# MatteoGiuseppetti/Hybrid-Autoencoder-MLP-Pipeline-for-Satellite-Image-Classification

Measured on AMD Instinct MI355X. Metric: EuroSAT 64x64 RGB images/sec (AE+MLP train step), higher is better.
Workload: dtype bf16; 1 GPU; BASELINE configs[2]: joint conv-AE + classification head train step (fwd, 35*MSE+CE, bwd, Adam), 64x64x3 inputs, 64-d latent, bf16 storage / fp32 accumulate; per_gpu_batch=512, global_batch=512, parallelism=single

## Files before the change

### hybrid-autoencoder-mlp-pipeline-for-satellite-image-classification_amd/csrc/eae_ctx.h

```cpp
#pragma once
#include "eae_internal.h"
#include "eae_args.h"
#include <atomic>
#include <functional>
#include <vector>

#define RC(x) do { int rc__ = (x); if (rc__) return rc__; } while (0)

constexpr float BN_EPS = 1e-5f, BN_MOM = 0.1f;
const int ENC_C[5] = {3, 32, 64, 128, 256};
const int BN_C[7] = {32, 64, 128, 256, 128, 64, 32};
const int BN_GAMMA_IDX[7] = {2, 6, 10, 14, 22, 26, 30};
const int W3_PARAM[6] = {4, 8, 12, 20, 24, 28};
const int W3_A[6] = {64, 128, 256, 256, 128, 64};
const int W3_B[6] = {32, 64, 128, 128, 64, 32};
const int PREBN_BIAS[7] = {1, 5, 9, 13, 21, 25, 29};

struct eae_ctx {
  eae_config cfg;
  int H, W, L, C, Bm;
  int Cin = 3, CP = 4;
  int Lp = 0;
  bool lpad = false;
  float *gs_encw = nullptr, *gs_encb = nullptr, *gs_decw = nullptr, *gs_head = nullptr, *zstage = nullptr;
  size_t pk_w1p = 0, pk_bep = 0;
  bool fp8 = false;
  size_t pk8_p1[6] = {}, pk8_p2[6] = {};
  Fp8State* q = nullptr;
  float* bn_save = nullptr;
  long long Pn, K;
  long long poff[39], bnoff[15];
  float *P = nullptr, *G = nullptr, *M = nullptr, *V = nullptr, *bnrun = nullptr;
  long long* nbt = nullptr;
  long long adam_step = 0;
  bool packed = false;
  bool fwd_ready = false;
  bool fwd_eval_ready = false;
  bool has_enc = true, has_dec = true;
  int enc_ready = 0, dec_ready = 0;
  bool bwd_eval = false;
  bool prebn_dirty = false;
  int fwd_B = 0, fwd_head = 0;
  const float* fwd_x = nullptr;
  long long fwd_gen = 0;
  void* ws = nullptr;
  bf16_t *y[4], *u[3], *d0, *gy[4], *gu[3], *gd0, *g4;
  bf16_t *dyy[4], *dyu[3];
  float *z, *dz, *dzc, *coef_f[7], *coef_b[7], *stat, *wscratch, *fcpart, *msepart, *cepart, *headpart, *lossbuf;
  long long wscratch_floats, head_stride;
  uint8_t* pack = nullptr;
// ... 80 lines not shown
  bool clip_on() const { return clip_max != 0.f; }
  float* dyn = nullptr;
  static constexpr int PROF_RING = 64;
  bool prof_on = false;
  int prof_site = 0;
  int prof_n = 0;
  hipEvent_t prof_ev[3 * PROF_RING] = {};
  EaeProfHook prof_hook = {};
  long long act_elems(int lvl) const {
    return (long long)(H >> lvl) * (W >> lvl) * ENC_C[lvl];
  }
};

inline void invalidate_forward(eae_ctx* c) { c->fwd_ready = false; c->fwd_eval_ready = false; c->enc_ready = 0; c->dec_ready = 0; }
inline long long r4(long long n) { return (n + 3) & ~3LL; }
inline unsigned* poison_word(const eae_ctx* c) { return reinterpret_cast<unsigned*>(c->acc_base + c->poison_off); }
inline SrcDesc src_raw(const bf16_t* p) { SrcDesc s; s.p0 = p; s.p1 = nullptr; s.coef = nullptr; return s; }
inline SrcDesc src_bnrelu(const bf16_t* y, const float* coef) { SrcDesc s; s.p0 = y; s.p1 = nullptr; s.coef = coef; return s; }
inline SrcDesc src_bnbwd(const bf16_t* g, const bf16_t* y, const float* coef) { SrcDesc s; s.p0 = g; s.p1 = y; s.coef = coef; return s; }
inline SrcDesc src_f32(const float* p) { SrcDesc s; s.p0 = reinterpret_cast<const bf16_t*>(p); s.p1 = nullptr; s.coef = nullptr; return s; }

extern const unsigned EV_FLAGS;

void sq_push(eae_ctx* c, std::function<int(hipStream_t, float*)> f, int pin = -1);
void sq_fork(eae_ctx* c);
void take_sig(eae_ctx* c, ConvArgs& a);
int sq_commit(eae_ctx* c, hipStream_t st);
int fold_side2(eae_ctx* c);
int join_side_begin(eae_ctx* c, hipStream_t st, GateArgs* g);
int join_side(eae_ctx* c, hipStream_t st);
int streams_distinct(eae_ctx* c, hipStream_t user);
// ... 17 lines not shown
```

### hybrid-autoencoder-mlp-pipeline-for-satellite-image-classification_amd/csrc/eae_ctx.hip

```cpp
#include "eae_ctx.h"
#include <string>
#include <cstring>
#include <cstdlib>

static thread_local std::string g_err;
int eae_set_error(int code, const char* msg) { g_err = msg ? msg : "unknown error"; return code; }
extern "C" const char* eae_last_error(void) { return g_err.c_str(); }
extern "C" int eae_version(void) { return 100; }

const unsigned EV_FLAGS = hipEventDisableTiming | (getenv("EAE_EVENT_SYSTEM_FENCE") ? 0u : hipEventDisableSystemFence);

namespace {

int bands_of(const eae_config& c) { return c.in_channels == 0 ? 3 : c.in_channels; }

void param_sizes(const eae_config& c, long long* sz) {
  const long long P = (long long)(c.image_h / 16) * (c.image_w / 16), K = 256 * P, L = c.latent_dim, C = c.num_classes;
  const long long N = bands_of(c);
  const long long s[38] = {32 * 9 * N, 32, 32, 32, 64 * 32 * 9, 64, 64, 64, 128 * 64 * 9, 128, 128, 128, 256 * 128 * 9, 256, 256, 256,
                           L * K, L, K * L, K, 256 * 128 * 9, 128, 128, 128, 128 * 64 * 9, 64, 64, 64, 64 * 32 * 9, 32, 32, 32,
                           32 * 9 * N, N, 128 * L, 128, C * 128, C};
  for (int i = 0; i < 38; ++i) sz[i] = s[i];
}

// ... 126 lines not shown
  const long long LK = c->Lp * c->K;
  c->pk_we1 = pcarve(LK * 2); add(c->poff[16], c->pk_we1, LK, PACK_FC_ROWMAJOR_KPERM, c->Lp, 256, (int)c->Pn, 0);
  c->pk_we2 = pcarve(LK * 2); add(c->poff[16], c->pk_we2, LK, PACK_FC_TRANS_KPERM, c->Lp, 256, (int)c->Pn, 0);
  c->pk_wd1 = pcarve(LK * 2); add(c->poff[18], c->pk_wd1, LK, PACK_FC_ROWPERM, c->Lp, 256, (int)c->Pn, 0);
  c->pk_wd2 = pcarve(LK * 2); add(c->poff[18], c->pk_wd2, LK, PACK_FC_ROWPERM_TRANS, c->Lp, 256, (int)c->Pn, 0);
  for (int k = 0; k < 4; ++k) descs[descs.size() - 1 - k].lv = c->L;
  if (c->lpad) {
    c->pk_w1p = pcarve(128LL * c->Lp * 4); add(c->poff[34], c->pk_w1p, 128LL * c->Lp, PACK_PAD_COLS, c->Lp, 0, 0, 1); descs.back().lv = c->L;
    c->pk_bep = pcarve(c->Lp * 4); add(c->poff[17], c->pk_bep, c->Lp, PACK_PAD_COLS, c->Lp, 0, 0, 1); descs.back().lv = c->L;
  }
  c->pk_bd = pcarve(c->K * 4); add(c->poff[19], c->pk_bd, c->K, PACK_FC_ROWPERM, 1, 256, (int)c->Pn, 1);
  c->ndesc = (int)descs.size();
  std::vector<unsigned short> blkmap(descs.size() * 1024);
  c->blk_tot = eae_pack_assign_blocks(descs.data(), (int)descs.size(), blkmap.data(), (int)blkmap.size());
  c->pack_bytes = poffb;
  size_t o_pack = carve(poffb), o_desc = carve(descs.size() * sizeof(PackDesc)), o_q = carve(sizeof(Fp8State)), o_bns = carve(2048 * 4 + 64);
  size_t o_bmap = carve((size_t)(c->blk_tot > 0 ? c->blk_tot : 1) * sizeof(unsigned short));
  hipError_t e = hipMalloc(&c->ws, off);
  if (e != hipSuccess) { delete c; return eae_set_error(EAE_ERR_HIP, hipGetErrorString(e)); }
  uint8_t* b = static_cast<uint8_t*>(c->ws);
  for (int i = 0; i < 4; ++i) { c->y[i] = (bf16_t*)(b + o_y[i]); c->gy[i] = (bf16_t*)(b + o_gy[i]); }
  for (int i = 0; i < 3; ++i) {
    c->u[i] = (bf16_t*)(b + o_u[i]); c->gu[i] = (bf16_t*)(b + o_gu[i]);
    c->dyu[i] = ((dy_mask_env >> (4 + i)) & 1u) ? (bf16_t*)(b + o_dyu[i]) : nullptr;
  }
  c->dyy[0] = nullptr;
  for (int i = 1; i < 4; ++i) c->dyy[i] = ((dy_mask_env >> i) & 1u) ? (bf16_t*)(b + o_dyy[i]) : nullptr;
  c->d0 = (bf16_t*)(b + o_d0); c->gd0 = (bf16_t*)(b + o_gd0); c->g4 = (bf16_t*)(b + o_g4);
  c->z = (float*)(b + o_z); c->dz = (float*)(b + o_dz); c->dzc = (float*)(b + o_dzc);
  if (c->lpad) {
// ... 13 lines not shown
  c->sigwords = (unsigned*)(b + o_sig);
  c->q = (Fp8State*)(b + o_q);
  c->bn_save = (float*)(b + o_bns);
  {
    Fp8State h;
    eae_fp8_state_init(&h);
    hipError_t eq = hipMemcpy(c->q, &h, sizeof(h), hipMemcpyHostToDevice);
    if (eq != hipSuccess) { hipFree(c->ws); delete c; return eae_set_error(EAE_ERR_HIP, hipGetErrorString(eq)); }
  }
  const char* rcc = getenv("ROCPROF_COUNTER_COLLECTION");
  c->use_gates = getenv("EAE_FORK_EVENTS") == nullptr && !(rcc && atoi(rcc) != 0);
  if (const char* gt = getenv("EAE_GATE_TIMEOUT_MS")) c->gate_limit = (unsigned long long)(atof(gt) * 1e5);
  c->use_graph = getenv("EAE_GRAPH") != nullptr;
  e = hipMemcpy(c->descs_dev, descs.data(), descs.size() * sizeof(PackDesc), hipMemcpyHostToDevice);
  if (e == hipSuccess && c->blk_tot > 0) e = hipMemcpy(c->blkmap, blkmap.data(), (size_t)c->blk_tot * sizeof(unsigned short), hipMemcpyHostToDevice);
  if (e == hipSuccess) e = hipMemset(c->g4, 0, Bm * (size_t)c->H * c->W * c->CP * 2);
  if (e == hipSuccess && c->lpad) e = hipMemset(c->zstage, 0, Bm * (size_t)c->Lp * 4);
  if (e == hipSuccess) e = hipMemset(c->z, 0, Bm * (size_t)c->Lp * 4);
  if (e == hipSuccess) e = hipMemset(c->dz, 0, Bm * (size_t)c->Lp * 4);
  if (e == hipSuccess) e = hipMemset(c->acc_base, 0, c->acc_bytes);
  if (e == hipSuccess) e = hipMemset(c->sigwords, 0, 64);
  c->acc_clean = true; c->bwd_dirty = false;
  c->dy_mask = (getenv("EAE_DY_MASK") ? (unsigned)strtoul(getenv("EAE_DY_MASK"), nullptr, 0) : 0u) & 0x3cu;
  c->skip_wgrad = getenv("EAE_SKIP_WGRAD") != nullptr;
  c->nan_exact = (getenv("EAE_NAN_EXACT") && atoi(getenv("EAE_NAN_EXACT")) != 0) ? 1 : 0;
  c->fold_fwd = getenv("EAE_NO_FOLD_FWD") == nullptr;
  c->fold_bwd = getenv("EAE_NO_FOLD_BWD") == nullptr;
  if (e != hipSuccess) { hipFree(c->ws); delete c; return eae_set_error(EAE_ERR_HIP, hipGetErrorString(e)); }
  c->use_side = getenv("EAE_NO_SIDE_STREAM") == nullptr && cfg->side_streams >= 0;
  if (c->use_side) {
// ... 224 lines not shown
```

### hybrid-autoencoder-mlp-pipeline-for-satellite-image-classification_amd/csrc/eae_dp.hip

```cpp
#include "eae_ctx.h"
#include "eae_common.hip.h"
#include <chrono>
#include <cstring>
#include <cstdlib>
#include <future>
#include <memory>
#include <string>
#include <thread>
#include <dlfcn.h>
#include <rccl/rccl.h>
namespace {
struct RcclApi {
  void* h = nullptr;
  decltype(&ncclGetUniqueId) getUniqueId = nullptr;
  decltype(&ncclCommInitRank) commInitRank = nullptr;
  decltype(&ncclCommDestroy) commDestroy = nullptr;
  decltype(&ncclAllReduce) allReduce = nullptr;
  decltype(&ncclBroadcast) broadcast = nullptr;
  decltype(&ncclGetErrorString) getErrorString = nullptr;
  decltype(&ncclGroupStart) groupStart = nullptr;
  decltype(&ncclGroupEnd) groupEnd = nullptr;
  std::string err;
};
RcclApi* rccl_api() {
// ... 132 lines not shown
    EAE_HIP(hipEventRecord(c->ev_dp_done, c->dp_stream[0]));
  }
  if (grp) RCCL(r->groupStart(), "ncclGroupStart");
  {
    int rc = eae_dp_allreduce_bucket(c, st, 0, ov ? cut : total);
    if (!rc) {
      ncclResult_t e = r->allReduce(flag, flag, 2, ncclUint32, ncclMax, static_cast<ncclComm_t>(c->dp_comm), st);
      if (e != ncclSuccess) rc = rccl_fail(r, e, "ncclAllReduce (flag)");
    }
    if (grp) { ncclResult_t e = r->groupEnd(); if (!rc && e != ncclSuccess) rc = rccl_fail(r, e, "ncclGroupEnd"); }
    RC(rc);
  }
  if (ov) EAE_HIP(hipStreamWaitEvent(st, c->ev_dp_done, 0));
  RC(launch_adam(c, st, c->poff[38], lr, 0.f, 1.0f / (float)c->dp_world, flag, flag + 1));
  c->last_loss = nullptr;
  c->packed = false; c->acc_clean = true; c->bwd_dirty = false;
  return 0;
}
```

### hybrid-autoencoder-mlp-pipeline-for-satellite-image-classification_amd/csrc/eae_misc.h

```cpp
#pragma once
#include <hip/hip_runtime.h>
#include <stdint.h>

enum { PACK_COPY = 0, PACK_3x3_P1, PACK_3x3_P2, PACK_K27, PACK_DECONV4_JOINT, PACK_FC_ROWMAJOR_KPERM, PACK_FC_TRANS_KPERM,
       PACK_FC_ROWPERM, PACK_FC_ROWPERM_TRANS, PACK_KCP, PACK_PAD_COLS };

struct PackDesc {
  long long src_off;
  long long dst_off;
  long long count;
  int mode, d0, d1, d2;
  int out_f32;
  int lv;
  int q_layer;
  int blk0, nblk;
};

constexpr int FP8_AMAX_SLOTS = 64;
constexpr int FP8_AMAX_STRIDE = 32;
struct Fp8State {
  unsigned amax_act[6][FP8_AMAX_SLOTS * FP8_AMAX_STRIDE];
  unsigned amax_grad[6][FP8_AMAX_SLOTS * FP8_AMAX_STRIDE];
  unsigned amax_w[6][FP8_AMAX_SLOTS * FP8_AMAX_STRIDE];
  float s_act[6], s_grad[6], s_w[6];
// ... 36 lines not shown
                         void* pack_base, Fp8State* q = nullptr, unsigned* clear_word = nullptr);
int eae_launch_adam(hipStream_t st, float* p, const float* g, float* m, float* v, long long n, double lr, double b1, double b2,
                    double eps, double wd, long long step);
constexpr int EAE_CLIP_MAX_PARTS = 512;
struct EaeClip { const double* part; int nparts; float max_norm; float* norm_out; };
int eae_grad_sumsq_parts(long long n);
int eae_launch_grad_sumsq(hipStream_t st, const float* g, const long long* poff39, const long long* sizes38, double* part);
int eae_launch_adam_dyn(hipStream_t st, float* p, const float* g, float* m, float* v, long long n, double b1, double b2, double eps,
                        const float* dyn, const unsigned* bad = nullptr, const unsigned* bad2 = nullptr, float* nan_out = nullptr,
                        const EaeClip* clip = nullptr);
int eae_launch_set_dyn(hipStream_t st, float* dyn, double lr, double b1, double b2, double wd, long long step);
int eae_launch_adam_scaled(hipStream_t st, float* p, const float* g, float* m, float* v, long long n, double lr, double b1, double b2,
                           double eps, double wd, long long step, float gscale, void* zero_buf = nullptr, long long zero_bytes = 0,
                           const unsigned* bad = nullptr, const unsigned* bad2 = nullptr, float* nan_out = nullptr, int nan_fill = 0,
                           int max_blocks = 0 , const EaeClip* clip = nullptr);
int eae_launch_stage_bands(hipStream_t st, const void* src, int elem_bytes, long long N, int C, int H, int W, const long long* index, int B,
                           const float* divisor, float* out, int train, float std, unsigned long long seed, unsigned long long step,
                           const int* params, const float* noise);
int eae_launch_augment(hipStream_t st, const void* in_u8, float* out, int B, int H, int W, int train, float std, unsigned long long seed,
                       unsigned long long step, const int* params, const float* noise);

__device__ __forceinline__ void philox4(uint32_t c0, uint32_t c1, uint32_t c2, uint32_t c3, uint32_t k0, uint32_t k1, uint32_t* o) {
#pragma unroll
  for (int r = 0; r < 10; ++r) {
    uint32_t h0 = __umulhi(0xD2511F53u, c0), l0 = 0xD2511F53u * c0;
    uint32_t h1 = __umulhi(0xCD9E8D57u, c2), l1 = 0xCD9E8D57u * c2;
    uint32_t n0 = h1 ^ c1 ^ k0, n1 = l1, n2 = h0 ^ c3 ^ k1, n3 = l0;
    c0 = n0; c1 = n1; c2 = n2; c3 = n3;
    k0 += 0x9E3779B9u; k1 += 0xBB67AE85u;
  }
// ... 18 lines not shown
```

### hybrid-autoencoder-mlp-pipeline-for-satellite-image-classification_amd/csrc/eae_misc.hip

```cpp
#include "eae_internal.h"
#include "eae_common.hip.h"
#include "eae_misc.h"


__device__ __forceinline__ double wave_sum_f64(double v) {
#pragma unroll
  for (int o = 32; o >= 1; o >>= 1) v += __shfl_xor(v, o, 64);
  return v;
}
__device__ __forceinline__ void reduce_partials_ch(const float* __restrict__ part, int ntiles, int C, int ch, double* red,
                                                   double& a, double& b) {
  const int tid = threadIdx.x;
  const float* p1 = part + (size_t)ch * ntiles;
  const float* p2 = part + ((size_t)C + ch) * ntiles;
  double s1 = 0.0, s2 = 0.0;
  for (int t = tid; t < ntiles; t += 256) { s1 += (double)p1[t]; s2 += (double)p2[t]; }
  s1 = wave_sum_f64(s1); s2 = wave_sum_f64(s2);
  if ((tid & 63) == 0) { red[tid >> 6] = s1; red[4 + (tid >> 6)] = s2; }
  __syncthreads();
  a = ((red[0] + red[1]) + red[2]) + red[3];
  b = ((red[4] + red[5]) + red[6]) + red[7];
}

__global__ EAE_NO_PK __launch_bounds__(256) void bn_finalize_kernel(const float* __restrict__ part, int ntiles, int C, float count,
// ... 136 lines not shown
  const SignalArgs a = group_args<SignalArgs>(gz);
  if (threadIdx.x == 0 && blockIdx.x == 0) __hip_atomic_store(a.word, a.val, __ATOMIC_RELAXED, __HIP_MEMORY_SCOPE_AGENT);
}
int eae_launch_gate(hipStream_t st, const GateArgs& g) {
  eae_launch(gate_kernel, gate_kernel_g, dim3(1), dim3(64), 0, st, g);
  EAE_LAUNCH_CHECK();
  return 0;
}
int eae_launch_signal(hipStream_t st, unsigned* word, unsigned val) {
  const SignalArgs sa = {word, val};
  eae_launch(signal_kernel, signal_kernel_g, dim3(1), dim3(64), 0, st, sa);
  EAE_LAUNCH_CHECK();
  return 0;
}

__device__ __forceinline__ float pack_fetch(const PackDesc& d, const float* __restrict__ src, unsigned i) {
  const unsigned d0 = (unsigned)d.d0, d1 = (unsigned)d.d1, d2 = (unsigned)d.d2;
  switch (d.mode) {
    case PACK_3x3_P1: {
      unsigned b = i % d1, r = i / d1, tap = r % 9u, a = r / 9u;
      return src[(a * d1 + b) * 9u + tap];
    }
    case PACK_3x3_P2: {
      unsigned a = i % d0, r = i / d0, tap = r % 9u, b = r / 9u;
      return src[(a * d1 + b) * 9u + tap];
    }
    case PACK_K27: {
      unsigned k = i & 31u, a = i >> 5;
      if (k >= 27u) return 0.f;
      unsigned tap = k / 3u, c = k % 3u;
      return src[(a * 3u + c) * 9u + tap];
    }
    case PACK_KCP: {
      const unsigned KP = (9u * d2 + 31u) & ~31u, k = i % KP, a = i / KP, tap = k / d2, c = k % d2;
      if (tap >= 9u || c >= d1) return 0.f;
      return src[(a * d1 + c) * 9u + tap];
    }
    case PACK_DECONV4_JOINT: {
      int k = i & 127; int n = i >> 7;
      const int C = (int)d1;
      if (n >= 4 * C) return 0.f;
      int ph = n / C, co = n % C, nb = k >> 5, ci = k & 31;
      int py = ph >> 1, px = ph & 1, dy = nb >> 1, dx = nb & 1;
      int ky = py == 0 ? (dy == 0 ? 1 : -1) : (dy == 0 ? 2 : 0);
      int kx = px == 0 ? (dx == 0 ? 1 : -1) : (dx == 0 ? 2 : 0);
      if (ky < 0 || kx < 0) return 0.f;
      return src[(ci * C + co) * 9 + ky * 3 + kx];
    }
    case PACK_FC_ROWMAJOR_KPERM: {
      unsigned K = d1 * d2, k2 = i % K, r = i / K;
      if (r >= (unsigned)d.lv) return 0.f;
      unsigned c = k2 % d1, p = k2 / d1;
      return src[r * K + c * d2 + p];
    }
    case PACK_FC_TRANS_KPERM: {
      unsigned r = i % d0, k2 = i / d0, K = d1 * d2;
      if (r >= (unsigned)d.lv) return 0.f;
      unsigned c = k2 % d1, p = k2 / d1;
      return src[r * K + c * d2 + p];
    }
    case PACK_FC_ROWPERM: {
      unsigned l = i % d0, j2 = i / d0;
// ... 333 lines not shown
      adam_update(P[j], __builtin_fmaf(G[j], CLIP ? geff : gscale, wp), M[j], V[j], b1, b2, step_size, bc2_sqrt, eps);
    }
    reinterpret_cast<float4*>(p)[i] = pp;
    reinterpret_cast<float4*>(m)[i] = mm;
    reinterpret_cast<float4*>(v)[i] = vv;
  }
}
__global__ EAE_NO_PK __launch_bounds__(256) void adam_kernel(AdamArgs a) { adam_body<false>(a); }
__global__ EAE_NO_PK __launch_bounds__(256) void adam_kernel_g(GroupPack<AdamArgs> p, int gz) { adam_body<false>(group_args<AdamArgs>(gz)); }
__global__ EAE_NO_PK __launch_bounds__(256) void adam_clip_kernel(AdamClipArgs a) { adam_body<true>(a.a, &a.c); }
__global__ EAE_NO_PK __launch_bounds__(256) void adam_clip_kernel_g(GroupPack<AdamClipArgs> p, int gz) {
  const AdamClipArgs a = group_args<AdamClipArgs>(gz);
  adam_body<true>(a.a, &a.c);
}

struct GradNormArgs { const float* g; double* part; unsigned n4; int ntail; unsigned tail[38]; };
__device__ __forceinline__ EAE_NO_PK void grad_sumsq_body(const GradNormArgs& a) {
#pragma clang fp contract(off)
  __shared__ double lds4[4];
  const unsigned T = gridDim.x * 256u, t = blockIdx.x * 256u + threadIdx.x, n4 = a.n4;
  const float4* __restrict__ g4 = reinterpret_cast<const float4*>(a.g);
  double acc = 0.0;
  for (unsigned i0 = t; i0 < n4; i0 += 4u * T) {
    float4 q[4];
#pragma unroll
    for (int u = 0; u < 4; ++u) {
      const unsigned i = i0 + (unsigned)u * T;
      q[u] = g4[i < n4 ? i : n4 - 1];
    }
#pragma unroll
// ... 249 lines not shown
```

### hybrid-autoencoder-mlp-pipeline-for-satellite-image-classification_amd/csrc/eae_step.hip

```cpp
#include "eae_ctx.h"
#include <cmath>
#include <cstdlib>

namespace {

static void prof_hook_begin(void* u, hipStream_t st) {
  eae_ctx* c = static_cast<eae_ctx*>(u);
  hipEventRecord(c->prof_ev[3 * c->prof_n], st);
}
static void prof_hook_end(void* u, hipStream_t st) {
  eae_ctx* c = static_cast<eae_ctx*>(u);
  hipEventRecord(c->prof_ev[3 * c->prof_n + 1], st);
  hipEventRecord(c->prof_ev[3 * c->prof_n + 2], st);
  c->prof_n++;
}
static const EaeProfHook* prof_hook_for(eae_ctx* c, int site) {
  if (!(c->prof_on && c->prof_site == site && c->prof_n < eae_ctx::PROF_RING && !c->capturing)) return nullptr;
  c->prof_hook = EaeProfHook{prof_hook_begin, prof_hook_end, c};
  return &c->prof_hook;
}
struct ProfBracket {
  eae_ctx* c; hipStream_t st; bool on;
  ProfBracket(eae_ctx* c_, int site, hipStream_t st_) : c(c_), st(st_) {
    on = c->prof_on && c->prof_site == site && c->prof_n < eae_ctx::PROF_RING && !c->capturing;
// ... 131 lines not shown
int run_head(eae_ctx* c, hipStream_t st, int B, const long long* labels, float* logits, bool want_grad, const float* dlogits_in,
             bool count_valid = false) {
  HeadArgs h = HeadArgs();
  h.dlogits_in = dlogits_in;
  h.z = c->z; h.w1 = c->lpad ? (const float*)(c->pack + c->pk_w1p) : c->P + c->poff[34]; h.b1 = c->P + c->poff[35]; h.w2 = c->P + c->poff[36]; h.b2 = c->P + c->poff[37];
  h.labels = labels; h.B = B; h.L = c->Lp; h.C = c->C; h.inv_batch = 1.0f / (float)B;
  h.logits = logits; h.dz = c->dzc; h.grad_part = want_grad ? c->headpart : nullptr; h.grad_stride = c->head_stride;
  h.loss_part = c->cepart;
  if (c->wce()) return eae_launch_head_w(st, h, c->class_w, c->ignore_index, count_valid ? c->valid_acc : nullptr);
  return eae_launch_head(st, h);
}

}

int ensure_packed(eae_ctx* c, hipStream_t st) {
  if (c->packed) return 0;
  RC(eae_launch_pack_flat(st, c->descs_dev, c->blkmap, 0, c->blk_tot, c->P, c->pack, c->fp8 ? c->q : nullptr, poison_word(c)));
  c->packed = true;
  return 0;
}

int prep_accumulators(eae_ctx* c, hipStream_t st, bool train) {
  if (!train || !c->fold_fwd) return 0;
  if (!c->acc_clean || c->capturing) { EAE_HIP(eae_memset_async(c->acc_base, 0, c->acc_bytes, st)); c->bwd_dirty = false; }
  c->acc_clean = false;
  return 0;
}

int copy_latent_out(eae_ctx* c, hipStream_t st, float* dst, const float* src_padded, int B) {
  if (!c->lpad) { EAE_HIP(hipMemcpyAsync(dst, src_padded, (size_t)B * c->L * 4, hipMemcpyDeviceToDevice, st)); return 0; }
  EAE_HIP(hipMemcpy2DAsync(dst, (size_t)c->L * 4, src_padded, (size_t)c->Lp * 4, (size_t)c->L * 4, B, hipMemcpyDeviceToDevice, st));
// ... 437 lines not shown
  EAE_HIP(hipDeviceSynchronize());
  Fp8State h;
  EAE_HIP(hipMemcpy(&h, c->q, sizeof(h), hipMemcpyDeviceToHost));
  for (int i = 0; i < 6; ++i) { out18[i] = h.s_act[i]; out18[6 + i] = h.s_grad[i]; out18[12 + i] = h.s_w[i]; }
  return 0;
}

int clip_prepare(eae_ctx* c, hipStream_t st, EaeClip* clip) {
  RC(eae_launch_grad_sumsq(st, c->G, c->poff, c->psize, c->clip_part));
  clip->part = c->clip_part; clip->nparts = eae_grad_sumsq_parts(c->poff[38]); clip->max_norm = c->clip_max; clip->norm_out = c->clip_out;
  return 0;
}
int launch_adam(eae_ctx* c, hipStream_t st, long long n, float lr, float wd, float grad_scale, const unsigned* bad, const unsigned* bad2) {
  EaeClip clip;
  if (c->clip_on()) RC(clip_prepare(c, st, &clip));
  return eae_launch_adam_scaled(st, c->P, c->G, c->M, c->V, n, lr, 0.9, 0.999, 1e-8, wd, c->adam_step, grad_scale, c->acc_base,
                                (long long)c->poison_off, bad ? bad : c->sigwords + 8, bad2 ? bad2 : poison_word(c), c->last_loss, c->nan_exact,
                                0, c->clip_on() ? &clip : nullptr);
}
int optimizer_step(eae_ctx* c, hipStream_t st, float lr, float wd, float grad_scale, const unsigned* bad, const unsigned* bad2) {
  if (!c || !c->P || !c->G || !c->M || !c->V) return eae_set_error(EAE_ERR_STATE, "adam: parameter, gradient and moment arenas must be bound");
  c->adam_step += 1;
  const int rc = launch_adam(c, st, c->poff[38], lr, wd, grad_scale, bad, bad2);
  c->last_loss = nullptr;
  c->packed = false; c->acc_clean = (rc == 0); c->bwd_dirty = !c->acc_clean;
  return rc;
}
extern "C" int eae_adam_step(eae_ctx* c, void* stream, float lr, float weight_decay) { return eae_adam_step_scaled(c, stream, lr, weight_decay, 1.0f); }

extern "C" int eae_ae_grad_step_begin(eae_ctx* c, void* stream, const eae_step_io* io) {
  RC(check_io(c, io, true));
  hipStream_t st = (hipStream_t)stream;
  RC(forward_impl(c, st, io, true));
  return backward_impl(c, st, io, nullptr, 1);
}
extern "C" int eae_ae_grad_step_end(eae_ctx* c, void* stream) {
  if (!c || !c->fwd_ready) return eae_set_error(EAE_ERR_STATE, "grad_step_end without grad_step_begin");
  eae_step_io io = eae_step_io();
  io.x = c->fwd_x; io.B = c->fwd_B; io.train = 1; io.head = c->fwd_head;
  int rc = backward_impl(c, (hipStream_t)stream, &io, nullptr, 2);
// ... 2 lines not shown
}
extern "C" int eae_adam_step_scaled(eae_ctx* c, void* stream, float lr, float weight_decay, float grad_scale) {
  return optimizer_step(c, (hipStream_t)stream, lr, weight_decay, grad_scale);
}

int train_step_eager(eae_ctx* c, hipStream_t st, const eae_step_io* io, float lr) {
  RC(streams_distinct(c, st));
  int rc = forward_impl(c, st, io, true);
  if (!rc) rc = backward_impl(c, st, io);
  if (!rc) {
    c->adam_step += 1;
    rc = launch_adam(c, st, c->poff[38], lr, 0.f, 1.0f);
    if (rc) c->adam_step -= 1;
  }
  c->last_loss = nullptr;
  c->packed = false; c->acc_clean = (rc == 0); c->bwd_dirty = !c->acc_clean;
  return rc;
}

extern "C" int eae_ae_train_step(eae_ctx* c, void* stream, const eae_step_io* io, float lr) {
  RC(check_io(c, io, true));
  if (!c->M || !c->V) return eae_set_error(EAE_ERR_STATE, "adam: moment arenas must be bound");
  hipStream_t user = (hipStream_t)stream, st = user;
  const bool graph_ok = c->use_graph && (c->use_side || user != nullptr) && c->fold_fwd && c->fold_bwd && !c->prof_on && !c->packed && io->logits == nullptr && io->z == nullptr;
  if (graph_ok && user == nullptr) {
    st = c->own_main;
    EAE_HIP(hipEventRecord(c->ev_in, user));
    EAE_HIP(hipStreamWaitEvent(st, c->ev_in, 0));
  }
  struct Rejoin {
    eae_ctx* c; hipStream_t user, st;
// ... 112 lines not shown
```

Baseline: 1.091 million images/s.

## Fuse Adam update with bf16 weight repacking into one tiled kernel

Adds a fused optimizer kernel that walks the parameter arena in per-tensor tiles, applies the Adam update, and writes the bf16 packed and permuted weight layouts (conv 3x3, FC, deconv, KCP) straight from LDS. The next step's `ensure_packed` then only repacks the leftover descriptors, or skips packing entirely. The poison/clear word now alternates parity so the fused kernel can clear the next step's flag. This removes a separate pack pass that re-read the fp32 parameters. In exchange the Adam pass uses tiled, less contiguous memory access and has a more complex block plan. It runs only when CUDA-graph capture is off, which is the default.

After: 1.101 million images/s (median of 6 runs). Within noise of the previous version (+1.0%).

```diff
diff --git a/hybrid-autoencoder-mlp-pipeline-for-satellite-image-classification_amd/csrc/eae_ctx.h b/hybrid-autoencoder-mlp-pipeline-for-satellite-image-classification_amd/csrc/eae_ctx.h
--- a/hybrid-autoencoder-mlp-pipeline-for-satellite-image-classification_amd/csrc/eae_ctx.h
+++ b/hybrid-autoencoder-mlp-pipeline-for-satellite-image-classification_amd/csrc/eae_ctx.h
@@ -33,7 +33,20 @@
   float *P = nullptr, *G = nullptr, *M = nullptr, *V = nullptr, *bnrun = nullptr;
   long long* nbt = nullptr;
   long long adam_step = 0;
-  bool packed = false;
+  struct PackState {
+    bool all = false, cov = false;
+    PackState& operator=(bool b) { all = cov = b; return *this; }
+    operator bool() const { return all; }
+  } packed;
+  bool fused_opt = true;
+  bool opt_was_fused = false;
+  FusedJob* fjobs_dev = nullptr;
+  unsigned short* fblkmap = nullptr;
+  int fblk_tot = 0;
+  PackDesc* descs_rest = nullptr;
+  unsigned short* blkmap_rest = nullptr;
+  int blk_rest = 0;
+  int poison_par = 0;
   bool fwd_ready = false;
   bool fwd_eval_ready = false;
   bool has_enc = true, has_dec = true;
@@ -144,7 +157,13 @@
 
 inline void invalidate_forward(eae_ctx* c) { c->fwd_ready = false; c->fwd_eval_ready = false; c->enc_ready = 0; c->dec_ready = 0; }
 inline long long r4(long long n) { return (n + 3) & ~3LL; }
-inline unsigned* poison_word(const eae_ctx* c) { return reinterpret_cast<unsigned*>(c->acc_base + c->poison_off); }
+inline unsigned* poison_word(const eae_ctx* c, int other = 0) { return reinterpret_cast<unsigned*>(c->acc_base + c->poison_off) + (c->poison_par ^ other); }
+inline void packs_after_optimizer(eae_ctx* c, int rc) {
+  const bool keep = rc == 0 && c->opt_was_fused && c->packed.cov;
+  c->packed = false;
+  if (keep) { c->packed.cov = true; c->packed.all = c->blk_rest == 0; }
+  c->opt_was_fused = false;
+}
 inline SrcDesc src_raw(const bf16_t* p) { SrcDesc s; s.p0 = p; s.p1 = nullptr; s.coef = nullptr; return s; }
 inline SrcDesc src_bnrelu(const bf16_t* y, const float* coef) { SrcDesc s; s.p0 = y; s.p1 = nullptr; s.coef = coef; return s; }
 inline SrcDesc src_bnbwd(const bf16_t* g, const bf16_t* y, const float* coef) { SrcDesc s; s.p0 = g; s.p1 = y; s.coef = coef; return s; }
diff --git a/hybrid-autoencoder-mlp-pipeline-for-satellite-image-classification_amd/csrc/eae_ctx.hip b/hybrid-autoencoder-mlp-pipeline-for-satellite-image-classification_amd/csrc/eae_ctx.hip
--- a/hybrid-autoencoder-mlp-pipeline-for-satellite-image-classification_amd/csrc/eae_ctx.hip
+++ b/hybrid-autoencoder-mlp-pipeline-for-satellite-image-classification_amd/csrc/eae_ctx.hip
@@ -164,6 +164,46 @@
   std::vector<unsigned short> blkmap(descs.size() * 1024);
   c->blk_tot = eae_pack_assign_blocks(descs.data(), (int)descs.size(), blkmap.data(), (int)blkmap.size());
   c->pack_bytes = poffb;
+  const bool fc_fused = !c->lpad && (long long)c->Lp * (256 / 64) * (c->Pn / 64) < 1024;
+  std::vector<FusedJob> fjobs;
+  std::vector<PackDesc> drest;
+  {
+    auto job = [&](int kind, int tensor, long long dst0, long long dst1, int d0, int d1, int d2) {
+      FusedJob j = FusedJob();
+      j.kind = kind; j.src_off = c->poff[tensor]; j.n4 = (c->poff[tensor + 1] - c->poff[tensor]) / 4; j.dst0 = dst0; j.dst1 = dst1; j.d0 = d0; j.d1 = d1; j.d2 = d2;
+      fjobs.push_back(j);
+    };
+    int plain_from = 0;
+    auto plain_until = [&](int tensor) {
+      if (tensor > plain_from) {
+        FusedJob j = FusedJob();
+        j.kind = FJ_PLAIN; j.src_off = c->poff[plain_from]; j.n4 = (c->poff[tensor] - c->poff[plain_from]) / 4;
+        fjobs.push_back(j);
+      }
+      plain_from = tensor + 1;
+    };
+    for (int t = 0; t < 38; ++t) {
+      int w3 = -1;
+      for (int i = 0; i < 6; ++i) if (W3_PARAM[i] == t) w3 = i;
+      if (t == 0) { plain_until(t); job(FJ_KCP, t, (long long)c->pk_c1, 0, 32, c->Cin, c->CP); }
+      else if (w3 >= 0) { plain_until(t); job(FJ_W3, t, (long long)c->pk_p1[w3], (long long)c->pk_p2[w3], W3_A[w3], W3_B[w3], 0); }
+      else if (t == 16 && fc_fused) { plain_until(t); job(FJ_ENCFC, t, (long long)c->pk_we1, (long long)c->pk_we2, c->Lp, 256, (int)c->Pn); }
+      else if (t == 18 && fc_fused) { plain_until(t); job(FJ_DECFC, t, (long long)c->pk_wd1, (long long)c->pk_wd2, c->Lp, 256, (int)c->Pn); }
+      else if (t == 19) { plain_until(t); job(FJ_BDPERM, t, (long long)c->pk_bd, 0, 1, 256, (int)c->Pn); }
+      else if (t == 32) { plain_until(t); job(FJ_DECONV4, t, (long long)c->pk_d4j, (long long)c->pk_d4k, 32, c->Cin, c->CP); }
+    }
+    plain_until(38);
+    for (const PackDesc& d : descs) {
+      const bool fc = d.mode == PACK_FC_ROWMAJOR_KPERM || d.mode == PACK_FC_TRANS_KPERM || ((d.mode == PACK_FC_ROWPERM || d.mode == PACK_FC_ROWPERM_TRANS) && !d.out_f32);
+      if (d.q_layer >= 0 || d.mode == PACK_PAD_COLS || (fc && !fc_fused)) drest.push_back(d);
+    }
+  }
+  std::vector<unsigned short> fblkmap(fjobs.size() * 1024), blkmap_rest(drest.size() * 1024 + 1);
+  c->fblk_tot = eae_fused_assign_blocks(fjobs.data(), (int)fjobs.size(), fblkmap.data(), (int)fblkmap.size());
+  c->blk_rest = drest.empty() ? 0 : eae_pack_assign_blocks(drest.data(), (int)drest.size(), blkmap_rest.data(), (int)blkmap_rest.size());
+  if (c->fblk_tot <= 0 || c->blk_rest < 0) { delete c; return eae_set_error(EAE_ERR_STATE, "create: no tile plan for the fused optimizer"); }
+  size_t o_fjobs = carve(fjobs.size() * sizeof(FusedJob)), o_fbmap = carve((size_t)c->fblk_tot * sizeof(unsigned short));
+  size_t o_drest = carve((drest.size() + 1) * sizeof(PackDesc)), o_bmrest = carve((size_t)(c->blk_rest + 1) * sizeof(unsigned short));
   size_t o_pack = carve(poffb), o_desc = carve(descs.size() * sizeof(PackDesc)), o_q = carve(sizeof(Fp8State)), o_bns = carve(2048 * 4 + 64);
   size_t o_bmap = carve((size_t)(c->blk_tot > 0 ? c->blk_tot : 1) * sizeof(unsigned short));
   hipError_t e = hipMalloc(&c->ws, off);
@@ -207,6 +247,13 @@
   c->use_graph = getenv("EAE_GRAPH") != nullptr;
   e = hipMemcpy(c->descs_dev, descs.data(), descs.size() * sizeof(PackDesc), hipMemcpyHostToDevice);
   if (e == hipSuccess && c->blk_tot > 0) e = hipMemcpy(c->blkmap, blkmap.data(), (size_t)c->blk_tot * sizeof(unsigned short), hipMemcpyHostToDevice);
+  c->fjobs_dev = (FusedJob*)(b + o_fjobs); c->fblkmap = (unsigned short*)(b + o_fbmap);
+  c->descs_rest = (PackDesc*)(b + o_drest); c->blkmap_rest = (unsigned short*)(b + o_bmrest);
+  if (e == hipSuccess) e = hipMemcpy(c->fjobs_dev, fjobs.data(), fjobs.size() * sizeof(FusedJob), hipMemcpyHostToDevice);
+  if (e == hipSuccess) e = hipMemcpy(c->fblkmap, fblkmap.data(), (size_t)c->fblk_tot * sizeof(unsigned short), hipMemcpyHostToDevice);
+  if (e == hipSuccess && c->blk_rest > 0) e = hipMemcpy(c->descs_rest, drest.data(), drest.size() * sizeof(PackDesc), hipMemcpyHostToDevice);
+  if (e == hipSuccess && c->blk_rest > 0) e = hipMemcpy(c->blkmap_rest, blkmap_rest.data(), (size_t)c->blk_rest * sizeof(unsigned short), hipMemcpyHostToDevice);
+  c->fused_opt = getenv("EAE_NO_FUSED_OPT") == nullptr || atoi(getenv("EAE_NO_FUSED_OPT")) == 0;
   if (e == hipSuccess) e = hipMemset(c->g4, 0, Bm * (size_t)c->H * c->W * c->CP * 2);
   if (e == hipSuccess && c->lpad) e = hipMemset(c->zstage, 0, Bm * (size_t)c->Lp * 4);
   if (e == hipSuccess) e = hipMemset(c->z, 0, Bm * (size_t)c->Lp * 4);
diff --git a/hybrid-autoencoder-mlp-pipeline-for-satellite-image-classification_amd/csrc/eae_dp.hip b/hybrid-autoencoder-mlp-pipeline-for-satellite-image-classification_amd/csrc/eae_dp.hip
--- a/hybrid-autoencoder-mlp-pipeline-for-satellite-image-classification_amd/csrc/eae_dp.hip
+++ b/hybrid-autoencoder-mlp-pipeline-for-satellite-image-classification_amd/csrc/eae_dp.hip
@@ -170,6 +170,6 @@
   if (ov) EAE_HIP(hipStreamWaitEvent(st, c->ev_dp_done, 0));
   RC(launch_adam(c, st, c->poff[38], lr, 0.f, 1.0f / (float)c->dp_world, flag, flag + 1));
   c->last_loss = nullptr;
-  c->packed = false; c->acc_clean = true; c->bwd_dirty = false;
+  packs_after_optimizer(c, 0); c->acc_clean = true; c->bwd_dirty = false;
   return 0;
 }
diff --git a/hybrid-autoencoder-mlp-pipeline-for-satellite-image-classification_amd/csrc/eae_misc.h b/hybrid-autoencoder-mlp-pipeline-for-satellite-image-classification_amd/csrc/eae_misc.h
--- a/hybrid-autoencoder-mlp-pipeline-for-satellite-image-classification_amd/csrc/eae_misc.h
+++ b/hybrid-autoencoder-mlp-pipeline-for-satellite-image-classification_amd/csrc/eae_misc.h
@@ -74,6 +74,21 @@
                            double eps, double wd, long long step, float gscale, void* zero_buf = nullptr, long long zero_bytes = 0,
                            const unsigned* bad = nullptr, const unsigned* bad2 = nullptr, float* nan_out = nullptr, int nan_fill = 0,
                            int max_blocks = 0 , const EaeClip* clip = nullptr);
+enum { FJ_PLAIN = 0, FJ_W3, FJ_ENCFC, FJ_DECFC, FJ_BDPERM, FJ_KCP, FJ_DECONV4 };
+struct FusedJob {
+  long long src_off;
+  long long n4;
+  long long dst0, dst1;
+  int kind, d0, d1, d2;
+  int tp;
+  unsigned ntiles;
+  int blk0, nblk;
+};
+int eae_fused_assign_blocks(FusedJob* jobs_host, int njobs, unsigned short* blkmap_host, int blkmap_cap);
+int eae_launch_fused_opt(hipStream_t st, float* p, const float* g, float* m, float* v, long long n, double lr, double b1, double b2, double eps,
+                         double wd, long long step, float gscale, void* zero_buf, long long zero_bytes, const unsigned* bad, const unsigned* bad2,
+                         float* nan_out, int nan_fill, const EaeClip* clip, const FusedJob* jobs_dev, const unsigned short* blkmap_dev, int nblocks,
+                         void* pack_base, unsigned* clear_word);
 int eae_launch_stage_bands(hipStream_t st, const void* src, int elem_bytes, long long N, int C, int H, int W, const long long* index, int B,
                            const float* divisor, float* out, int train, float std, unsigned long long seed, unsigned long long step,
                            const int* params, const float* noise);
diff --git a/hybrid-autoencoder-mlp-pipeline-for-satellite-image-classification_amd/csrc/eae_misc.hip b/hybrid-autoencoder-mlp-pipeline-for-satellite-image-classification_amd/csrc/eae_misc.hip
--- a/hybrid-autoencoder-mlp-pipeline-for-satellite-image-classification_amd/csrc/eae_misc.hip
+++ b/hybrid-autoencoder-mlp-pipeline-for-satellite-image-classification_amd/csrc/eae_misc.hip
@@ -174,6 +174,21 @@
   return 0;
 }
 
+__device__ __forceinline__ int kcp_src_index(unsigned i, unsigned C, unsigned CP) {
+  const unsigned KP = (9u * CP + 31u) & ~31u, k = i % KP, a = i / KP, tap = k / CP, c = k % CP;
+  if (tap >= 9u || c >= C) return -1;
+  return (int)((a * C + c) * 9u + tap);
+}
+__device__ __forceinline__ int d4j_src_index(unsigned i, int C) {
+  int k = i & 127; int n = i >> 7;
+  if (n >= 4 * C) return -1;
+  int ph = n / C, co = n % C, nb = k >> 5, ci = k & 31;
+  int py = ph >> 1, px = ph & 1, dy = nb >> 1, dx = nb & 1;
+  int ky = py == 0 ? (dy == 0 ? 1 : -1) : (dy == 0 ? 2 : 0);
+  int kx = px == 0 ? (dx == 0 ? 1 : -1) : (dx == 0 ? 2 : 0);
+  if (ky < 0 || kx < 0) return -1;
+  return (ci * C + co) * 9 + ky * 3 + kx;
+}
 __device__ __forceinline__ float pack_fetch(const PackDesc& d, const float* __restrict__ src, unsigned i) {
   const unsigned d0 = (unsigned)d.d0, d1 = (unsigned)d.d1, d2 = (unsigned)d.d2;
   switch (d.mode) {
@@ -192,20 +207,12 @@
       return src[(a * 3u + c) * 9u + tap];
     }
     case PACK_KCP: {
-      const unsigned KP = (9u * d2 + 31u) & ~31u, k = i % KP, a = i / KP, tap = k / d2, c = k % d2;
-      if (tap >= 9u || c >= d1) return 0.f;
-      return src[(a * d1 + c) * 9u + tap];
+      const int s = kcp_src_index(i, d1, d2);
+      return s < 0 ? 0.f : src[s];
     }
     case PACK_DECONV4_JOINT: {
-      int k = i & 127; int n = i >> 7;
-      const int C = (int)d1;
-      if (n >= 4 * C) return 0.f;
-      int ph = n / C, co = n % C, nb = k >> 5, ci = k & 31;
-      int py = ph >> 1, px = ph & 1, dy = nb >> 1, dx = nb & 1;
-      int ky = py == 0 ? (dy == 0 ? 1 : -1) : (dy == 0 ? 2 : 0);
-      int kx = px == 0 ? (dx == 0 ? 1 : -1) : (dx == 0 ? 2 : 0);
-      if (ky < 0 || kx < 0) return 0.f;
-      return src[(ci * C + co) * 9 + ky * 3 + kx];
+      const int s = d4j_src_index(i, (int)d1);
+      return s < 0 ? 0.f : src[s];
     }
     case PACK_FC_ROWMAJOR_KPERM: {
       unsigned K = d1 * d2, k2 = i % K, r = i / K;
@@ -569,6 +576,247 @@
   adam_body<true>(a.a, &a.c);
 }
 
+struct FusedOptArgs { AdamArgs a; ClipArgs c; const FusedJob* jobs; const unsigned short* blkmap; uint8_t* pack; unsigned* clear_word; int clip; };
+static_assert(sizeof(FusedOptArgs) <= 480, "the grouped twin carries 8 members' blocks in one launch");
+struct OptK { float* p; const float* g; float* m; float* v; float b1, b2, step_size, bc2_sqrt, eps, wd, geff; bool nan; };
+struct TileGeo { size_t s4; unsigned r0, c0, p0, n0, n1, sh; };
+template <int KIND> __device__ __forceinline__ EAE_NO_PK size_t tile_addr(const TileGeo& t, unsigned idx) {
+  if constexpr (KIND == FJ_W3) {
+    const unsigned row = idx / 36u, q = idx - row * 36u;
+    return t.s4 + (((size_t)(t.r0 + row) * t.n0 + t.c0) * 9u) / 4u + q;
+  } else if constexpr (KIND == FJ_ENCFC) {
+    const unsigned row = idx >> t.sh, q = idx & ((1u << t.sh) - 1u), ri = row >> 4, ci = row & 15u;
+    return t.s4 + ((size_t)(t.r0 + ri) * t.n0 + (size_t)(t.c0 + ci) * t.n1 + t.p0) / 4u + q;
+  } else if constexpr (KIND == FJ_DECFC) {
+    const unsigned row = idx >> 4, q = idx & 15u, ci = row >> 2, pi = row & 3u;
+    return t.s4 + (((size_t)(t.c0 + ci) * t.n1 + t.p0 + pi) * t.n0 + t.r0) / 4u + q;
+  } else if constexpr (KIND == FJ_BDPERM) {
+    const unsigned ci = idx >> 2, q = idx & 3u;
+    return t.s4 + ((size_t)(t.c0 + ci) * t.n1 + t.p0) / 4u + q;
+  } else {
+    return t.s4 + idx;
+  }
+}
+template <int KIND> __device__ __forceinline__ EAE_NO_PK void opt_tile(const OptK& k, unsigned n4t, const TileGeo& t, unsigned short* lds) {
+#pragma clang fp contract(off)
+  float4* __restrict__ p4 = reinterpret_cast<float4*>(k.p); const float4* __restrict__ g4 = reinterpret_cast<const float4*>(k.g);
+  float4* __restrict__ m4 = reinterpret_cast<float4*>(k.m); float4* __restrict__ v4 = reinterpret_cast<float4*>(k.v);
+  const float4 nn = make_float4(__builtin_nanf(""), __builtin_nanf(""), __builtin_nanf(""), __builtin_nanf(""));
+  for (unsigned base = 0; base < n4t; base += 1024u) {
+    float4 pp[4], gg[4], mm[4], vv[4];
+    size_t at[4];
+#pragma unroll
+    for (int u = 0; u < 4; ++u) {
+      const unsigned idx = base + (unsigned)u * 256u + threadIdx.x;
+      at[u] = 0; pp[u] = gg[u] = mm[u] = vv[u] = nn;
+      if (idx < n4t) {
+        at[u] = tile_addr<KIND>(t, idx);
+        if (!k.nan) { pp[u] = p4[at[u]]; gg[u] = g4[at[u]]; mm[u] = m4[at[u]]; vv[u] = v4[at[u]]; }
+      }
+    }
+#pragma unroll
+    for (int u = 0; u < 4; ++u) {
+      const unsigned idx = base + (unsigned)u * 256u + threadIdx.x;
+      if (idx >= n4t) continue;
+      if (!k.nan) {
+        float* P = &pp[u].x; float* G = &gg[u].x; float* M = &mm[u].x; float* V = &vv[u].x;
+#pragma unroll
+        for (int j = 0; j < 4; ++j) {
+          const float wp = k.wd * P[j];
+          adam_update(P[j], __builtin_fmaf(G[j], k.geff, wp), M[j], V[j], k.b1, k.b2, k.step_size, k.bc2_sqrt, k.eps);
+        }
+      }
+      p4[at[u]] = pp[u]; m4[at[u]] = mm[u]; v4[at[u]] = vv[u];
+      if constexpr (KIND == FJ_BDPERM) reinterpret_cast<float4*>(lds)[idx] = pp[u];
+      else if constexpr (KIND != FJ_PLAIN)
+        *reinterpret_cast<uint2*>(lds + (size_t)idx * 4u) = make_uint2(pack2(pp[u].x, pp[u].y), pack2(pp[u].z, pp[u].w));
+    }
+  }
+}
+__device__ __forceinline__ uint2 lds_gather4(const unsigned short* lds, unsigned i0, unsigned stride) {
+  return make_uint2((unsigned)lds[i0] | ((unsigned)lds[i0 + stride] << 16), (unsigned)lds[i0 + 2u * stride] | ((unsigned)lds[i0 + 3u * stride] << 16));
+}
+__device__ __forceinline__ EAE_NO_PK void fused_opt_body(const FusedOptArgs& fa) {
+  __shared__ __align__(16) unsigned short lds[16384];
+  const AdamArgs& aa = fa.a;
+  const unsigned tid = threadIdx.x;
+  for (long i = (long)blockIdx.x * 256 + tid; i < aa.zn16; i += (long)gridDim.x * 256) aa.zbuf[i] = make_uint4(0, 0, 0, 0);
+  if (fa.clear_word != nullptr && blockIdx.x == 0 && tid == 0) *fa.clear_word = 0u;
+  const bool stale = aa.bad != nullptr && __hip_atomic_load(aa.bad, __ATOMIC_RELAXED, __HIP_MEMORY_SCOPE_AGENT) != 0u;
+  bool diverged = aa.bad2 != nullptr && __hip_atomic_load(aa.bad2, __ATOMIC_RELAXED, __HIP_MEMORY_SCOPE_AGENT) != 0u;
+  float geff = aa.gscale;
+  if (fa.clip) {
+    const ClipCoef cc = clip_coef(fa.c, aa.gscale);
+    diverged = diverged || !cc.finite;
+    geff = aa.gscale * cc.coef;
+  }
+  bool nanm = false;
+  if (stale || diverged) {
+    if (aa.nan_out != nullptr && blockIdx.x == 0 && tid < 3) aa.nan_out[tid] = __builtin_nanf("");
+    if (!(aa.nan_fill && diverged && !stale)) return;
+    nanm = true;
+  }
+  const OptK k = {aa.p, aa.g, aa.m, aa.v, aa.b1, aa.b2, aa.step_size, aa.bc2_sqrt, aa.eps, aa.wd, geff, nanm};
+  const FusedJob j = fa.jobs[fa.blkmap[blockIdx.x]];
+  const unsigned bx = blockIdx.x - (unsigned)j.blk0, nb = (unsigned)j.nblk;
+  bf16_t* q0 = reinterpret_cast<bf16_t*>(fa.pack + j.dst0);
+  bf16_t* q1 = reinterpret_cast<bf16_t*>(fa.pack + j.dst1);
+  TileGeo t = TileGeo();
+  t.s4 = (size_t)(j.src_off >> 2);
+  switch (j.kind) {
+    case FJ_W3: {
+      const unsigned A = (unsigned)j.d0, B = (unsigned)j.d1, nbt = B / 16u;
+      t.n0 = B;
+      for (unsigned tl = bx; tl < j.ntiles; tl += nb) {
+        t.r0 = (tl / nbt) * 16u; t.c0 = (tl % nbt) * 16u;
+        __syncthreads();
+        opt_tile<FJ_W3>(k, 576u, t, lds);
+        __syncthreads();
+        for (unsigned i = tid; i < 576u; i += 256u) {
+          const unsigned bq = i & 3u, r = i >> 2, tap = r % 9u, ar = r / 9u;
+          *reinterpret_cast<uint2*>(q0 + ((size_t)(t.r0 + ar) * 9u + tap) * B + t.c0 + bq * 4u) = lds_gather4(lds, ar * 144u + bq * 36u + tap, 9u);
+        }
+        for (unsigned i = tid; i < 576u; i += 256u) {
+          const unsigned aq = i & 3u, r = i >> 2, tap = r % 9u, br = r / 9u;
+          *reinterpret_cast<uint2*>(q1 + ((size_t)(t.c0 + br) * 9u + tap) * A + t.r0 + aq * 4u) = lds_gather4(lds, aq * 576u + br * 9u + tap, 144u);
+        }
+      }
+      break;
+    }
+    case FJ_ENCFC: {
+      const unsigned R = (unsigned)j.d0, Cc = (unsigned)j.d1, P = (unsigned)j.d2, K = Cc * P, tp = (unsigned)j.tp, tpl = tp == 64u ? 6u : 4u;
+      const unsigned np = P / tp, nc = Cc / 16u;
+      t.n0 = K; t.n1 = P; t.sh = tpl - 2u;
+      for (unsigned tl = bx; tl < j.ntiles; tl += nb) {
+        t.p0 = (tl % np) * tp; t.c0 = ((tl / np) % nc) * 16u; t.r0 = (tl / (np * nc)) * 16u;
+        __syncthreads();
+        opt_tile<FJ_ENCFC>(k, 64u * tp, t, lds);
+        __syncthreads();
+        for (unsigned i = tid; i < 64u * tp; i += 256u) {
+          const unsigned cq = i & 3u, r = i >> 2, pi = r & (tp - 1u), ri = r >> tpl;
+          *reinterpret_cast<uint2*>(q0 + (size_t)(t.r0 + ri) * K + (size_t)(t.p0 + pi) * Cc + t.c0 + cq * 4u) = lds_gather4(lds, (ri * 16u + cq * 4u) * tp + pi, tp);
+        }
+        for (unsigned i = tid; i < 64u * tp; i += 256u) {
+          const unsigned rq = i & 3u, r = i >> 2, ci = r & 15u, pi = r >> 4;
+          *reinterpret_cast<uint2*>(q1 + ((size_t)(t.p0 + pi) * Cc + t.c0 + ci) * R + t.r0 + rq * 4u) = lds_gather4(lds, (rq * 64u + ci) * tp + pi, 16u * tp);
+        }
+      }
+      break;
+    }
+    case FJ_DECFC: {
+      const unsigned L = (unsigned)j.d0, Cc = (unsigned)j.d1, P = (unsigned)j.d2, J = Cc * P, nl = L / 64u, np = P / 4u;
+      t.n0 = L; t.n1 = P;
+      for (unsigned tl = bx; tl < j.ntiles; tl += nb) {
+        t.r0 = (tl % nl) * 64u; t.p0 = ((tl / nl) % np) * 4u; t.c0 = (tl / (nl * np)) * 16u;
+        __syncthreads();
+        opt_tile<FJ_DECFC>(k, 1024u, t, lds);
+        __syncthreads();
+        for (unsigned i = tid; i < 1024u; i += 256u) {
+          const unsigned lq = i & 15u, row = i >> 4, ci = row >> 2, pi = row & 3u;
+          *reinterpret_cast<uint2*>(q0 + ((size_t)(t.p0 + pi) * Cc + t.c0 + ci) * L + t.r0 + lq * 4u) = *reinterpret_cast<const uint2*>(lds + i * 4u);
+        }
+        for (unsigned i = tid; i < 1024u; i += 256u) {
+          const unsigned cq = i & 3u, pi = (i >> 2) & 3u, li = i >> 4;
+          *reinterpret_cast<uint2*>(q1 + (size_t)(t.r0 + li) * J + (size_t)(t.p0 + pi) * Cc + t.c0 + cq * 4u) = lds_gather4(lds, (cq * 16u + pi) * 64u + li, 256u);
+        }
+      }
+      break;
+    }
+    case FJ_BDPERM: {
+      const unsigned Cc = (unsigned)j.d1, P = (unsigned)j.d2, np = P / 16u;
+      const float* lf = reinterpret_cast<const float*>(lds);
+      float* qf = reinterpret_cast<float*>(fa.pack + j.dst0);
+      t.n1 = P;
+      for (unsigned tl = bx; tl < j.ntiles; tl += nb) {
+        t.p0 = (tl % np) * 16u; t.c0 = (tl / np) * 64u;
+        __syncthreads();
+        opt_tile<FJ_BDPERM>(k, 256u, t, lds);
+        __syncthreads();
+        const unsigned cq = tid & 15u, pi = tid >> 4, l0 = cq * 64u + pi;
+        *reinterpret_cast<float4*>(qf + (size_t)(t.p0 + pi) * Cc + t.c0 + cq * 4u) = make_float4(lf[l0], lf[l0 + 16u], lf[l0 + 32u], lf[l0 + 48u]);
+      }
+      break;
+    }
+    case FJ_KCP:
+    case FJ_DECONV4: {
+      if (bx != 0) break;
+      opt_tile<FJ_KCP>(k, (unsigned)j.n4, t, lds);
+      __syncthreads();
+      const unsigned C = (unsigned)j.d1, CP = (unsigned)j.d2, KP = (9u * CP + 31u) & ~31u;
+      if (j.kind == FJ_DECONV4) {
+        for (unsigned i = tid; i < CP * 128u; i += 256u) {
+          unsigned short e[4];
+#pragma unroll
+          for (unsigned q = 0; q < 4; ++q) { const int s = d4j_src_index(i * 4u + q, (int)C); e[q] = s < 0 ? (unsigned short)0 : lds[s]; }
+          *reinterpret_cast<uint2*>(q0 + (size_t)i * 4u) = make_uint2((unsigned)e[0] | ((unsigned)e[1] << 16), (unsigned)e[2] | ((unsigned)e[3] << 16));
+        }
+      }
+      bf16_t* qk = j.kind == FJ_DECONV4 ? q1 : q0;
+      for (unsigned i = tid; i < 8u * KP; i += 256u) {
+        unsigned short e[4];
+#pragma unroll
+        for (unsigned q = 0; q < 4; ++q) { const int s = kcp_src_index(i * 4u + q, C, CP); e[q] = s < 0 ? (unsigned short)0 : lds[s]; }
+        *reinterpret_cast<uint2*>(qk + (size_t)i * 4u) = make_uint2((unsigned)e[0] | ((unsigned)e[1] << 16), (unsigned)e[2] | ((unsigned)e[3] << 16));
+      }
+      break;
+    }
+    default: {
+      for (unsigned tl = bx; tl < j.ntiles; tl += nb) {
+        const long long rem = j.n4 - (long long)tl * 1024;
+        t.s4 = (size_t)(j.src_off >> 2) + (size_t)tl * 1024u;
+        opt_tile<FJ_PLAIN>(k, rem < 1024 ? (unsigned)rem : 1024u, t, lds);
+      }
+      break;
+    }
+  }
+}
+__global__ EAE_NO_PK __launch_bounds__(256) void fused_opt_kernel(FusedOptArgs a) { fused_opt_body(a); }
+__global__ EAE_NO_PK __launch_bounds__(256) void fused_opt_kernel_g(GroupPack<FusedOptArgs> p, int gz) { fused_opt_body(group_args<FusedOptArgs>(gz)); }
+
+int eae_fused_assign_blocks(FusedJob* jobs, int njobs, unsigned short* blkmap, int cap) {
+  int tot = 0;
+  for (int i = 0; i < njobs; ++i) {
+    FusedJob& j = jobs[i];
+    long long tiles = 1;
+    j.tp = 0;
+    switch (j.kind) {
+      case FJ_PLAIN: tiles = (j.n4 + 1023) / 1024; break;
+      case FJ_W3: if (j.d0 % 16 || j.d1 % 16) return -1; tiles = (long long)(j.d0 / 16) * (j.d1 / 16); break;
+      case FJ_ENCFC:
+        if (j.d0 % 16 || j.d1 % 16 || j.d2 % 16) return -1;
+        j.tp = j.d2 % 64 == 0 ? 64 : 16;
+        tiles = (long long)(j.d0 / 16) * (j.d1 / 16) * (j.d2 / j.tp);
+        break;
+      case FJ_DECFC: if (j.d0 % 64 || j.d1 % 16 || j.d2 % 4) return -1; tiles = (long long)(j.d0 / 64) * (j.d1 / 16) * (j.d2 / 4); break;
+      case FJ_BDPERM: if (j.d1 % 64 || j.d2 % 16) return -1; tiles = (long long)(j.d1 / 64) * (j.d2 / 16); break;
+      case FJ_KCP: case FJ_DECONV4: if (j.n4 * 4 > 16384) return -1; break;
+      default: return -1;
+    }
+    if (tiles < 1 || tiles >= (1LL << 31)) return -1;
+    j.ntiles = (unsigned)tiles;
+    j.blk0 = tot; j.nblk = (int)(tiles > 1024 ? 1024 : tiles);
+    for (int b = 0; b < j.nblk; ++b) { if (tot + b >= cap) return -1; blkmap[tot + b] = (unsigned short)i; }
+    tot += j.nblk;
+  }
+  return tot;
+}
+int eae_launch_fused_opt(hipStream_t st, float* p, const float* g, float* m, float* v, long long n, double lr, double b1, double b2, double eps,
+                         double wd, long long step, float gscale, void* zero_buf, long long zero_bytes, const unsigned* bad, const unsigned* bad2,
+                         float* nan_out, int nan_fill, const EaeClip* clip, const FusedJob* jobs_dev, const unsigned short* blkmap_dev, int nblocks,
+                         void* pack_base, unsigned* clear_word) {
+  if (n % 4) return eae_set_error(-2, "adam: arena length must be a multiple of 4");
+  if (!jobs_dev || !blkmap_dev || nblocks <= 0 || !pack_base || clear_word == bad2) return eae_set_error(-2, "fused optimizer: no tile plan");
+  const double bc1 = 1.0 - pow(b1, (double)step), bc2 = 1.0 - pow(b2, (double)step);
+  FusedOptArgs fa = FusedOptArgs();
+  fa.a = {p, g, m, v, (long)(n / 4), (float)b1, (float)b2, (float)(lr / bc1), (float)sqrt(bc2), (float)eps, (float)wd, gscale,
+          (uint4*)zero_buf, (long)(zero_bytes / 16), bad, bad2, nan_out, nan_fill};
+  if (clip) { fa.c = {clip->part, clip->nparts, clip->max_norm, clip->norm_out}; fa.clip = 1; }
+  fa.jobs = jobs_dev; fa.blkmap = blkmap_dev; fa.pack = (uint8_t*)pack_base; fa.clear_word = clear_word;
+  eae_launch(fused_opt_kernel, fused_opt_kernel_g, dim3(nblocks), dim3(256), 0, st, fa);
+  EAE_LAUNCH_CHECK();
+  return 0;
+}
+
 struct GradNormArgs { const float* g; double* part; unsigned n4; int ntail; unsigned tail[38]; };
 __device__ __forceinline__ EAE_NO_PK void grad_sumsq_body(const GradNormArgs& a) {
 #pragma clang fp contract(off)
diff --git a/hybrid-autoencoder-mlp-pipeline-for-satellite-image-classification_amd/csrc/eae_step.hip b/hybrid-autoencoder-mlp-pipeline-for-satellite-image-classification_amd/csrc/eae_step.hip
--- a/hybrid-autoencoder-mlp-pipeline-for-satellite-image-classification_amd/csrc/eae_step.hip
+++ b/hybrid-autoencoder-mlp-pipeline-for-satellite-image-classification_amd/csrc/eae_step.hip
@@ -169,7 +169,12 @@
 }
 
 int ensure_packed(eae_ctx* c, hipStream_t st) {
-  if (c->packed) return 0;
+  if (c->packed.all) return 0;
+  if (c->packed.cov) {
+    RC(eae_launch_pack_flat(st, c->descs_rest, c->blkmap_rest, 0, c->blk_rest, c->P, c->pack, c->fp8 ? c->q : nullptr, nullptr));
+    c->packed = true;
+    return 0;
+  }
   RC(eae_launch_pack_flat(st, c->descs_dev, c->blkmap, 0, c->blk_tot, c->P, c->pack, c->fp8 ? c->q : nullptr, poison_word(c)));
   c->packed = true;
   return 0;
@@ -637,6 +642,16 @@
 int launch_adam(eae_ctx* c, hipStream_t st, long long n, float lr, float wd, float grad_scale, const unsigned* bad, const unsigned* bad2) {
   EaeClip clip;
   if (c->clip_on()) RC(clip_prepare(c, st, &clip));
+  c->opt_was_fused = false;
+  if (c->fused_opt && !c->use_graph && !c->capturing && n == c->poff[38]) {
+    const unsigned* b2 = bad2 ? bad2 : poison_word(c);
+    RC(eae_launch_fused_opt(st, c->P, c->G, c->M, c->V, n, lr, 0.9, 0.999, 1e-8, wd, c->adam_step, grad_scale, c->acc_base, (long long)c->poison_off,
+                            bad ? bad : c->sigwords + 8, b2, c->last_loss, c->nan_exact, c->clip_on() ? &clip : nullptr, c->fjobs_dev, c->fblkmap,
+                            c->fblk_tot, c->pack, poison_word(c, 1)));
+    c->poison_par ^= 1;
+    c->opt_was_fused = true;
+    return 0;
+  }
   return eae_launch_adam_scaled(st, c->P, c->G, c->M, c->V, n, lr, 0.9, 0.999, 1e-8, wd, c->adam_step, grad_scale, c->acc_base,
                                 (long long)c->poison_off, bad ? bad : c->sigwords + 8, bad2 ? bad2 : poison_word(c), c->last_loss, c->nan_exact,
                                 0, c->clip_on() ? &clip : nullptr);
@@ -646,7 +661,7 @@
   c->adam_step += 1;
   const int rc = launch_adam(c, st, c->poff[38], lr, wd, grad_scale, bad, bad2);
   c->last_loss = nullptr;
-  c->packed = false; c->acc_clean = (rc == 0); c->bwd_dirty = !c->acc_clean;
+  packs_after_optimizer(c, rc); c->acc_clean = (rc == 0); c->bwd_dirty = !c->acc_clean;
   return rc;
 }
 extern "C" int eae_adam_step(eae_ctx* c, void* stream, float lr, float weight_decay) { return eae_adam_step_scaled(c, stream, lr, weight_decay, 1.0f); }
@@ -679,7 +694,7 @@
     if (rc) c->adam_step -= 1;
   }
   c->last_loss = nullptr;
-  c->packed = false; c->acc_clean = (rc == 0); c->bwd_dirty = !c->acc_clean;
+  packs_after_optimizer(c, rc); c->acc_clean = (rc == 0); c->bwd_dirty = !c->acc_clean;
   return rc;
 }
 
```
